# moldyn/Clustering

Measured on AMD Instinct MI355X. Metric: frame-pairs/s (density pop+nn), higher is better.
Workload: dtype f32 (Gram form on two fp16 pieces per coordinate on the f16 MFMA pipe, f32 accumulate, as a classifier with a guard band; undecided pairs re-checked in canonical f32)

## Files before the change

clustering_amd/csrc/dc_mfma.hip:

```cpp
#include "dc_mfma_kernels.hpp"
#include "dc_against.hpp"
#include "dc_against_nn.hpp"

#include <algorithm>
#include <cstring>
#include <atomic>
#include <mutex>

#ifndef DC_STEP_MASK
#define DC_STEP_MASK 0xFFFFu
#endif

namespace dc {

namespace {

#include "dc_mfma32.hpp"

__global__ void colsum_kernel(const float* __restrict__ coords, uint32_t n_rows, uint32_t D,
                              double* __restrict__ sums) {
  __shared__ double part[kMaxCols];
  if (threadIdx.x < (uint32_t)kMaxCols) part[threadIdx.x] = 0.0;
  __syncthreads();
  const uint32_t nthreads = gridDim.x * blockDim.x;
// ... 880 lines not shown
    const char* v;
    if ((v = env("DC_POP_SYM"))) w.pop_sym = v[0] != '0';
    if ((v = env("DC_POP_SHARED"))) w.pop_shared = atoi(v);
    if ((v = env("DC_NN_SHARED"))) w.nn_shared = atoi(v);
    w.waves_per_group = one_of_124(env("DC_WAVES_PER_GROUP"), 0);
    if ((v = env("DC_NN_COOP"))) w.nn_coop = atoi(v);
    if ((v = env("DC_NN_RHO"))) w.nn_rho = v[0] != '0';
    if ((v = env("DC_WAVE_TARGET"))) w.wave_target = (uint32_t)atoi(v);
    if ((v = env("DC_SHARE_FLOOR"))) w.share_floor = (uint32_t)atoi(v);
    if ((v = env("DC_POP_COMPONENTS"))) w.components = v[0] != '0';
    w.pop_cell_frames = (v = env("DC_POP_CELL_FRAMES")) ? (float)atof(v) : kPopCellFrames;
    w.nn_cell_frames = (v = env("DC_NN_CELL_FRAMES")) ? (float)atof(v) : kNnCellFrames;
    if ((v = env("DC_NN_FE_BITS"))) w.nn_fe_bits = atoi(v);
    w.mfma32_wpb = (uint32_t)one_of_124(env("DC_MFMA32_WPB"), 1);
    if ((v = env("DC_MFMA32_CHUNKS"))) w.mfma32_chunks = (uint32_t)atoi(v);
    return w;
  }();
  return sw;
}

static float cell_frames(bool nn) { return nn ? sweep_switches().nn_cell_frames : sweep_switches().pop_cell_frames; }
static float nn_cell_frames() { return cell_frames(true); }

int mfma_prepare(const float* d_coords, uint32_t n_rows, uint32_t n_cols, void* d_ws, hipStream_t stream,
                 bool stats_valid, bool pruned, const float* d_fe) {
  char* p = (char*)d_ws;
  const uint32_t cookie = data_cookie(d_coords, n_rows, n_cols);
  if (stats_valid) {
    const Layout L = make_layout(n_rows, n_cols);
    const size_t total = (size_t)n_rows * n_cols;
    const uint32_t B = (uint32_t)std::max<size_t>(1, std::min<size_t>(kClaimBlocks, (total + 1023) / 1024));
    unsigned long long* tab = (unsigned long long*)(p + L.fixed_end);
    const bool nn_reuse = pruned && d_fe != nullptr;
// ... 1163 lines not shown
```

clustering_amd/csrc/dc_mfma.hpp:

```cpp
#pragma once
#include "dc_common.hpp"

namespace dc {

struct EdgeSink {
  uint2* edges;
  unsigned long long* count;
  unsigned long long capacity;
  const uint32_t* comp;
  const uint32_t* rank;
  unsigned long long* best;
};
enum SinkMode { kSinkNone = 0, kSinkPairs = 1, kSinkMinEdge = 2 };

struct SweepSwitches {
  bool pop_sym = true;
  int pop_shared = -1;
  int nn_shared = -1;
  int waves_per_group = 0;
  int nn_coop = -1;
  bool nn_rho = true;
  uint32_t wave_target = 0;
  uint32_t share_floor = 0;
  bool components = true;
  float pop_cell_frames = 0.0f;
  float nn_cell_frames = 0.0f;
  int nn_fe_bits = -1;
  uint32_t mfma32_wpb = 1;
  uint32_t mfma32_chunks = 0;
};
const SweepSwitches& sweep_switches();

enum PopForm {
  kPopWave,
  kPopWaveSym,
  kPopPairs,
  kPopMinEdge,
  kPopShared,
  kPopSharedSym,
  kPopMsym,
  kPopMulti,
};
enum NnForm {
  kNnWave,
  kNnShared,
};
// ... 131 lines not shown
```

clustering_amd/csrc/dc_mfma_kernels.hpp:

```cpp
#pragma once
#include "dc_mfma.hpp"
#include "dc_credit.hpp"
#include "dc_rho_gap.hpp"
#include "dc_wide_prune.hpp"

#include <assert.h>
#include <float.h>
#include <math.h>
#include <stdlib.h>

#include <type_traits>

namespace dc {

namespace {

typedef float f32x16 __attribute__((ext_vector_type(16)));
typedef short s16x8 __attribute__((ext_vector_type(8)));

constexpr int kMaxCols = 64;
constexpr int kConstSlots = 2;
constexpr int kPieceGroups = 3;
constexpr int nm_for(int n_cols) { return (kPieceGroups * n_cols + kConstSlots + 15) / 16; }
constexpr int kMaxMfma = nm_for(kMaxCols);
// ... 175 lines not shown
  float cinv;
  int g, a, rounded;
};
constexpr uint32_t kHdrScale = 20;
constexpr uint32_t kHdrFp = 14;
constexpr uint32_t kHdrCookie = 28;
constexpr uint32_t kHdrMused = 31;
constexpr uint32_t kHdrOpen = 30;
constexpr uint32_t kHdrMfmaPop = 6, kHdrMfmaNn = 26;
constexpr uint32_t kHdrLayoutBad = 18;
constexpr uint32_t kHdrShares = 19;
constexpr uint32_t kHdrStatsBlocks = 25;
constexpr int kMfmaCtrPop = (kHdrMfmaPop - 2) / 2, kMfmaCtrNn = (kHdrMfmaNn - 4) / 2;
constexpr uint32_t kHdrShift = 32;
constexpr uint32_t kHdrMloc = 29;
constexpr int kMidShiftPop = 6, kConstShiftPop = 6, kConstShiftNn = 15;
constexpr float kThrCapPop = 1048576.0f;

__host__ __device__ inline Scale make_scale(const ScaleExp& e) {
  Scale s;
  s.sa = e.c;
  s.sb = e.c;
  s.s2 = e.s2;
  s.up = ldexpf(1.0f, e.g);
  s.dn = ldexpf(1.0f, -e.g);
  s.cinv = ldexpf(1.0f, -e.a);
  s.g = e.g;
  s.a = e.a;
  s.rounded = e.rounded;
  return s;
// ... 501 lines not shown
#pragma unroll
    for (int rr = 0; rr < NR; ++rr) {
      const uint32_t total = q[qt].cnt[rr] + (uint32_t)__shfl_xor((int)q[qt].cnt[rr], 32, 64);
      if (h == 0 && live && rr < n_rad) {
        if constexpr (M == kSelf) {
          const float dself = exact_d2(X.qcoords, n_cols, jq[qt], jq[qt]);
          pops[(size_t)rr * X.n_q + jq[qt]] = total + 1u - ((dself < rad2.v[rr]) ? 1u : 0u);
        } else {
          pops[(size_t)rr * X.n_q + jq[qt]] = total;
        }
      }
    }
  }
}

__device__ __forceinline__ uint32_t xcd_block(uint32_t n_blocks) {
  const uint32_t b = blockIdx.x, phys = b & 7u, idx = b >> 3;
  const uint32_t eighth = (phys + blockIdx.y) & 7u;
  const uint32_t n_full = n_blocks >> 3, rem = n_blocks & 7u;
  if (idx >= n_full + (eighth < rem ? 1u : 0u)) return 0xFFFFFFFFu;
  return eighth * n_full + min(eighth, rem) + idx;
}
inline uint32_t grid_x8(uint32_t n_blocks) { return (n_blocks + 7u) & ~7u; }

enum QueryMode { kQueryOwnOrder = 0, kQueryAll = 1 };

constexpr int kListCap = 512;
constexpr int kQueueCap = 4;
constexpr int kWaveQueue = 128;
constexpr int kSeedNeighbours = 4;

constexpr uint32_t kPopQueuePosBits = 24;
constexpr uint32_t kPopQueueMaxRows = 1u << kPopQueuePosBits;
static_assert(kMinEdgeMaxRows + kOrderPadRows == kPopQueueMaxRows, "min-edge sweeps take the queue path only");
static_assert(kOrderPadRows == (size_t)32 * kPadTiles, "pad positions of the orders");

__device__ __forceinline__ void emit_edge(const EdgeSink& sink, bool have, uint32_t pos_q, uint32_t pos_r) {
  const uint64_t m = __builtin_amdgcn_ballot_w64(have);
// ... 144 lines not shown
        if (e0 + 64u * j < total) dst[e0 + 64u * j] = v[j];
    }
  } else if (lane < 32) {
    const float* x = coords + (size_t)frame * n_cols;
    for (uint32_t k0 = 0; k0 < n_cols; k0 += 4) {
      float v[4];
#pragma unroll
      for (uint32_t j = 0; j < 4; ++j) v[j] = (live && k0 + j < n_cols) ? x[k0 + j] : 0.0f;
#pragma unroll
      for (uint32_t j = 0; j < 4; ++j)
        if (k0 + j < n_cols) dst[(uint32_t)lane * n_cols + k0 + j] = v[j];
    }
  }
}

template <int NM, int NR, int TQ, int MODE = kSinkNone, bool SYM = false>
__global__ __launch_bounds__(256, 2) void pop_pruned_kernel(
    const float* __restrict__ coords, uint32_t n_rows, uint32_t n_cols,
    const uint4* __restrict__ img_r, const float* __restrict__ norms_r,
    const uint32_t* __restrict__ perm_r, const float4* __restrict__ box_r,
    const float* __restrict__ coords_r, uint32_t T,
    const uint4* __restrict__ img_q, const float* __restrict__ norms_q,
    const uint32_t* __restrict__ perm_q, const float4* __restrict__ box_q, uint32_t n_q, QSeg q_seg,
    const uint32_t* __restrict__ hdr, unsigned long long* __restrict__ chain_counter, Rad2 rad2,
    int n_rad, uint32_t* __restrict__ pops, EdgeSink sink, CompView CV, uint32_t* __restrict__ pops_pos = nullptr) {
  static_assert(!SYM || (MODE == kSinkNone && NR == 1), "the symmetric sweep is the plain one-radius sweep");
  extern __shared__ __attribute__((aligned(16))) float pop_dyn_lds[];
  if (hdr[1] != 0) return;
  const int lane = threadIdx.x & 63, h = lane >> 5, c = lane & 31;
  const int wib = threadIdx.x >> 6;
  const uint32_t wpb = blockDim.x >> 6;
  uint32_t* lists_all = reinterpret_cast<uint32_t*>(pop_dyn_lds);
  float* pop_qrows_all = pop_dyn_lds + (size_t)wpb * kListCap;
  const uint32_t TQT = (n_q + 31) / 32;
  const uint32_t blk_unit = xcd_block((seg_groups((TQT + TQ - 1) / TQ, q_seg) + wpb - 1) / wpb);
  if (blk_unit == 0xFFFFFFFFu) return;
  const uint32_t wave = seg_group(blk_unit * wpb + wib, q_seg);
  const uint32_t chunk = blockIdx.y, n_chunks = gridDim.y;
  const uint32_t qt0 = wave * TQ;
  if (qt0 >= TQT) return;
  const uint32_t my_comp = CV.tile_comp_q[qt0];
  const uint32_t comp_lo = CV.range_r[2 * my_comp], comp_hi = CV.range_r[2 * my_comp + 1];
  uint32_t* list = lists_all + (size_t)wib * kListCap;
  float* qrows = pop_qrows_all + (size_t)wib * (TQ * 32) * n_cols;
  uint32_t* queues = reinterpret_cast<uint32_t*>(pop_qrows_all + (size_t)wpb * (TQ * 32) * n_cols) +
                     (size_t)wib * TQ * kQueueCap * 64;
  const bool use_queue = CV.n_pos <= kPopQueueMaxRows;
  constexpr bool kWaveWide = (MODE == kSinkNone) && (NR == 1) && (TQ * 32 <= 256) && (TQ * kQueueCap * 64 >= kWaveQueue + TQ * 32);
  uint32_t* fix_tab = queues + kWaveQueue;
  uint32_t qn = 0;
  uint32_t qcount[TQ];
  uint32_t comp_q[TQ], rank_q[TQ];
  unsigned long long edge_key[TQ];
// ... 339 lines not shown
        if (chunk == 0) {
          const float dself = exact_d2(coords, n_cols, jq[qt], jq[qt]);
          v += 1u - ((dself < rad2.v[rr]) ? 1u : 0u);
        }
        if constexpr (SYM)
          atomicAdd(&pops_pos[(qt0 + (uint32_t)qt) * 32u + (uint32_t)c], v);
        else if (n_chunks == 1)
          pops[(size_t)rr * n_rows + jq[qt]] = v;
        else
          atomicAdd(&pops[(size_t)rr * n_rows + jq[qt]], v);
      }
    }
  }
}


#include "dc_mfma_shared.hpp"
#include "dc_mfma_msym.hpp"

__device__ __forceinline__ void lexi_update(bool cond, float& bd, uint32_t& bj, float d,
                                            uint32_t j, uint32_t n_rows) {
  const bool take = cond & ((d < bd) | ((d == bd) & (j < bj) & (bj <= n_rows)));
  bd = take ? d : bd;
  bj = take ? j : bj;
}

struct NnQ {
  float m_nn, m_hd;
  float bd_nn, bd_hd;
  uint32_t bj_nn, bj_hd;
// ... 341 lines not shown
    const short one = live ? (short)const_a_bits(sc.a) : (short)0;
    b[0][0] = one;
    b[0][1] = one;
  }
}
template <int NM>
__device__ __forceinline__ void load_tile_folded(const uint4* __restrict__ img, uint32_t t, int lane, s16x8 (&a)[NM]) {
  const uint4* ip = img + (size_t)t * (NM * 64) + lane;
#pragma unroll
  for (int m = 0; m < NM; ++m) {
    const uint4 v = ip[m * 64];
    a[m] = __builtin_bit_cast(s16x8, v);
  }
}

template <int NM, int TQ, bool COOP = false>
__global__ __launch_bounds__(COOP ? 512 : 256, COOP ? 1 : 2) void nn_pruned_kernel(
    const float* __restrict__ coords, uint32_t n_rows, uint32_t n_cols,
    const float* __restrict__ fe, const uint4* __restrict__ img_r,
    const float* __restrict__ norms_r, const uint32_t* __restrict__ perm_r,
    const float4* __restrict__ box_r, const float4* __restrict__ box_t,
    const float2* __restrict__ rho_r, const float2* __restrict__ rho_t,
    const float2* __restrict__ ferange_r,
    const float* __restrict__ fe_c, const float* __restrict__ coords_c,
    const uint32_t* __restrict__ invpos_r, uint32_t T,
    const uint4* __restrict__ img_q, const float* __restrict__ norms_q,
    const uint32_t* __restrict__ perm_q, const float4* __restrict__ box_q, uint32_t n_q, QSeg q_seg,
    int full_range, float cell2,
    const uint32_t* __restrict__ hdr, unsigned long long* __restrict__ chain_counter,
    unsigned long long* __restrict__ merge64, uint32_t* __restrict__ nn_idx,
    float* __restrict__ nn_d2, uint32_t* __restrict__ hd_idx, float* __restrict__ hd_d2, CompView CV) {
  extern __shared__ __attribute__((aligned(16))) float nn_dyn_lds[];
  if (hdr[1] != 0) return;
  const int lane = threadIdx.x & 63, h = lane >> 5, c = lane & 31;
  const int wib = threadIdx.x >> 6;
  const uint32_t wpb = blockDim.x >> 6;
  uint32_t* lists_all = reinterpret_cast<uint32_t*>(nn_dyn_lds);
  float* qrows_all = nn_dyn_lds + (size_t)wpb * kListCap;
  const uint32_t TQT = (n_q + 31) / 32;
  const uint32_t blk_unit = xcd_block(COOP ? seg_groups((TQT + TQ - 1) / TQ, q_seg) : (seg_groups((TQT + TQ - 1) / TQ, q_seg) + wpb - 1) / wpb);
  if (blk_unit == 0xFFFFFFFFu) return;
  const uint32_t wave = seg_group(COOP ? blk_unit : blk_unit * wpb + wib, q_seg);
  const uint32_t chunk = COOP ? blockIdx.y * wpb + (uint32_t)wib : blockIdx.y, n_chunks = COOP ? gridDim.y * wpb : gridDim.y;
  const uint32_t qt0 = wave * TQ;
  if (qt0 >= TQT) return;
  const uint32_t my_comp = CV.tile_comp_q[qt0];
  const uint32_t comp_lo = CV.range_r[2 * my_comp], comp_hi = CV.range_r[2 * my_comp + 1];
  const float comp_cell = __uint_as_float(CV.comp[kCompFine + 4 * min(my_comp, (uint32_t)kMaxComp - 1u) + 2]);
  uint32_t* list = lists_all + (size_t)wib * kListCap;
  uint32_t* coop_base = lists_all + (size_t)wpb * kListCap;
  float* qrows = COOP ? reinterpret_cast<float*>(coop_base + (size_t)wpb * 2 * kWaveQueue + 8 * TQ * 32)
                      : qrows_all + (size_t)wib * (TQ * 32) * n_cols;
  uint32_t* queues = COOP ? coop_base + (size_t)wib * 2 * kWaveQueue
                          : reinterpret_cast<uint32_t*>(qrows_all + (size_t)wpb * (TQ * 32) * n_cols) +
                                (size_t)wib * (TQ * kQueueCap * 64 + 2 * TQ * 32);
  static_assert(TQ * kQueueCap * 64 >= 2 * kWaveQueue + 4 * TQ * 32, "candidate list + incumbents fit the queue region");
  uint2* cand = reinterpret_cast<uint2*>(queues);
  unsigned long long* best64 = reinterpret_cast<unsigned long long*>(COOP ? coop_base + (size_t)wpb * 2 * kWaveQueue : queues + 2 * kWaveQueue);
// ... 70 lines not shown
        for (uint32_t j = 0; j < 8; ++j) v[j] = (e0 + nthr * j < total) ? src[e0 + nthr * j] : 0.0f;
#pragma unroll
        for (uint32_t j = 0; j < 8; ++j)
          if (e0 + nthr * j < total) qrows[e0 + nthr * j] = v[j];
      }
    } else {
#pragma unroll
      for (int qt = 0; qt < TQ; ++qt) {
        if (((uint32_t)qt % wpb) != (uint32_t)wib) continue;
        const uint32_t tile = qt0 + qt, tl = tile < TQT ? tile : TQT - 1;
        stage_query_rows(qrows + (size_t)qt * 32 * n_cols, full_range ? coords_c + (size_t)tl * 32 * n_cols : nullptr, coords,
                         jq[qt], (livemask[qt] >> lane) & 1, n_cols, lane);
      }
    }
    __syncthreads();
    if (blockIdx.y == 0) {
#pragma unroll
      for (int qt = 0; qt < TQ; ++qt) {
        const bool live = (livemask[qt] >> lane) & 1;
        float bd_nn = FLT_MAX, bd_hd = FLT_MAX;
        uint32_t bj_nn = n_rows + 1, bj_hd = n_rows + 1;
        if (live) {
          const float* qrow = qrows + (qt * 32 + c) * n_cols;
          for (int k = 1 + wib; k <= kSeedNeighbours; k += (int)wpb) {
            const long long p2 = (long long)q[qt].spos + (h ? -k : k);
            if (p2 >= 0 && p2 < (long long)CV.n_pos && perm_r[p2] != kInvalidFrame) {
              const float d2c = dist2_canon_rt(qrow, 1, coords_c + (size_t)p2 * n_cols, 1, (int)n_cols);
              const uint32_t j = perm_r[p2];
              lexi_update(true, bd_nn, bj_nn, d2c, j, n_rows);
              lexi_update(fe_c[p2] < q[qt].feq, bd_hd, bj_hd, d2c, j, n_rows);
            }
// ... 488 lines not shown
      jq[qt] = perm_q[(qt0 + qt) * 32 + c];
      const unsigned long long w_nn = best64[qt * 32 + c], w_hd = best64[TQ * 32 + qt * 32 + c];
      if (n_chunks == 1) {
        nn_idx[jq[qt]] = (uint32_t)w_nn;
        nn_d2[jq[qt]] = __uint_as_float((uint32_t)(w_nn >> 32));
        hd_idx[jq[qt]] = (uint32_t)w_hd;
        hd_d2[jq[qt]] = __uint_as_float((uint32_t)(w_hd >> 32));
      } else {
        atomicMin(&merge64[jq[qt]], w_nn);
        atomicMin(&merge64[(size_t)n_rows + jq[qt]], w_hd);
      }
    }
  }
}

#include "dc_mfma_nn_shared.hpp"

__global__ void nn_merge_fill_kernel(unsigned long long* __restrict__ merge64, uint32_t n_rows) {
  const uint32_t i = blockIdx.x * blockDim.x + threadIdx.x;
  if (i < 2 * n_rows) merge64[i] = ((unsigned long long)__float_as_uint(FLT_MAX) << 32) | (n_rows + 1);
}

__global__ void nn_merge_unpack_kernel(const unsigned long long* __restrict__ merge64,
                                       const uint32_t* __restrict__ perm_q, uint32_t n_q,
                                       uint32_t n_rows, uint32_t tq, QSeg q_seg,
                                       uint32_t* __restrict__ nn_idx, float* __restrict__ nn_d2,
                                       uint32_t* __restrict__ hd_idx, float* __restrict__ hd_d2) {
  const uint32_t p = blockIdx.x * blockDim.x + threadIdx.x;
  if (p >= n_q) return;
  if (!seg_owns(p / (32u * tq), q_seg)) return;
// ... 34 lines not shown
  return (waves + 3) / 4;
}

template <int S, SweepMode M>
void pop_dispatch(const SweepArgs& X, uint32_t n_cols, uint32_t i_from, uint32_t i_to, const Rad2& rad2, uint32_t* pops,
                  hipStream_t s) {
  constexpr int kTQ = tq_full_for<S>;
  const dim3 grid(grid_for(i_from, i_to, kTQ)), block(256);
  sweep_timer_mark(0, true, s);
  hipLaunchKernelGGL((pop_mfma_kernel<S, 1, kTQ, M>), grid, block, 0, s, X, n_cols, i_from, i_to, rad2, 1, pops);
  sweep_timer_mark(0, false, s);
}

__global__ void box_by_share_kernel(const float4* __restrict__ box_r, uint32_t T, uint32_t n_chunks,
                                    float4* __restrict__ box_t, const float2* __restrict__ rho_r,
                                    float2* __restrict__ rho_t) {
  const uint32_t t = blockIdx.x * blockDim.x + threadIdx.x;
  if (t >= T) return;
  const uint32_t stride = (T + n_chunks - 1) / n_chunks;
  box_t[(size_t)(t % n_chunks) * stride + t / n_chunks] = box_r[t];
  if (rho_r) rho_t[(size_t)(t % n_chunks) * stride + t / n_chunks] = rho_r[t];
}

struct NnPrunedArgs {
  const uint4* img_r;
  const float* norms_r;
  const uint32_t* perm_r;
  const float4* box_r;
  float4* box_t;
  const float2* rho_r;
  float2* rho_t;
  const float2* ferange_r;
// ... 97 lines not shown
  if (sw.share_floor) share_floor = sw.share_floor;
  const uint32_t waves = (tiles + tq - 1) / tq;
  uint32_t r = waves >= target ? 1u : (target + waves - 1) / waves;
  const uint32_t by_share = ref_tiles / share_floor;
  const uint32_t cap = by_share < 64u ? by_share : 64u;
  r = r > cap ? cap : r;
  return r < 1u ? 1u : r;
}

template <class F>
void timed_launch(int kind, hipStream_t s, F&& launch) {
  sweep_timer_mark(kind, true, s);
  launch();
  sweep_timer_mark(kind, false, s);
}
inline void nn_shares_begin(const NnPrunedArgs& A, uint32_t n_rows, uint32_t T, uint32_t n_chunks, bool with_rho, hipStream_t s) {
  if (n_chunks > 1)
    hipLaunchKernelGGL(nn_merge_fill_kernel, dim3((2 * n_rows + 255) / 256), dim3(256), 0, s, A.merge64, n_rows);
  hipLaunchKernelGGL(box_by_share_kernel, dim3((T + 255) / 256), dim3(256), 0, s, A.box_r, T, n_chunks, A.box_t,
                     with_rho ? A.rho_r : (const float2*)nullptr, A.rho_t);
}
inline void nn_shares_end(const NnPrunedArgs& A, uint32_t n_rows, uint32_t n_chunks, uint32_t group_tiles,
                          uint32_t* nn_idx, float* nn_d2, uint32_t* hd_idx, float* hd_d2, hipStream_t s) {
  if (n_chunks <= 1) return;
  if (A.full_range)
    hipLaunchKernelGGL(nn_merge_unpack_rows_kernel, dim3((n_rows + 255) / 256), dim3(256), 0, s,
                       (const unsigned long long*)A.merge64, A.invpos_r, n_rows, group_tiles, A.q_seg, nn_idx, nn_d2,
                       hd_idx, hd_d2);
  else
    hipLaunchKernelGGL(nn_merge_unpack_kernel, dim3((A.n_q + 255) / 256), dim3(256), 0, s,
                       (const unsigned long long*)A.merge64, A.perm_q, A.n_q, n_rows, group_tiles, A.q_seg, nn_idx,
                       nn_d2, hd_idx, hd_d2);
}

template <int S>
// ... 28 lines not shown
          launch(std::integral_constant<int, kNbMin>{});
        else
          launch(std::integral_constant<int, kNbMax>{});
      } else {
        launch(std::integral_constant<int, kNbMax>{});
      }
      nn_shares_end(A, n_rows, n_chunks, 4u * TQV, nn_idx, nn_d2, hd_idx, hd_d2, s);
    }
    return;
  }
  constexpr int TQV = tq_nn(S);
  assert(pl.tq == (uint32_t)TQV);
  const uint32_t waves = seg_groups(((A.n_q + 31) / 32 + TQV - 1) / TQV, A.q_seg), tiles = waves * TQV;
  if (waves == 0) return;
  uint32_t n_chunks = pick_chunks(tiles, TQV, kNnWaveTargetPerWave, T, kNnShareFloor, (size_t)S * 1024 + 128);
  if (n_chunks >= pl.coop_shares) {
    n_chunks = (n_chunks + kNnCoopWaves - 1) / kNnCoopWaves * kNnCoopWaves;
    const size_t smem_c = sizeof(uint32_t) * (kNnCoopWaves * (kListCap + 2 * kWaveQueue) + 8 * TQV * 32) +
                          sizeof(float) * TQV * 32 * (size_t)n_cols;
    nn_shares_begin(A, n_rows, T, n_chunks, true, s);
    timed_launch(1, s, [&] {
      hipLaunchKernelGGL((nn_pruned_kernel<S, TQV, true>), dim3(grid_x8(waves), n_chunks / kNnCoopWaves), dim3(64 * kNnCoopWaves), smem_c, s,
                         coords, n_rows, n_cols, fe, A.img_r, A.norms_r, A.perm_r, A.box_r, (const float4*)A.box_t, A.rho_r,
                         (const float2*)(A.rho_r ? A.rho_t : nullptr), A.ferange_r, A.fe_c, A.coords_c, A.invpos_r, T, A.img_q, A.norms_q, A.perm_q, A.box_q, A.n_q, A.q_seg,
                         A.full_range, A.cell2, hdr, chain_counter, A.merge64, nn_idx, nn_d2, hd_idx, hd_d2, CV);
    });
  } else {
    const uint32_t wpb = pl.waves;
    const size_t smem = wpb * (sizeof(uint32_t) * kListCap + sizeof(float) * TQV * 32 * (size_t)n_cols +
                               sizeof(uint32_t) * (TQV * kQueueCap * 64 + 2 * TQV * 32));
    nn_shares_begin(A, n_rows, T, n_chunks, true, s);
    timed_launch(1, s, [&] {
      hipLaunchKernelGGL((nn_pruned_kernel<S, TQV>), dim3(grid_x8((waves + wpb - 1) / wpb), n_chunks), dim3(64 * wpb), smem, s,
                         coords, n_rows, n_cols, fe, A.img_r, A.norms_r, A.perm_r, A.box_r, (const float4*)A.box_t, A.rho_r,
                         (const float2*)(A.rho_r ? A.rho_t : nullptr), A.ferange_r, A.fe_c, A.coords_c, A.invpos_r, T, A.img_q, A.norms_q, A.perm_q, A.box_q, A.n_q, A.q_seg,
                         A.full_range, A.cell2, hdr, chain_counter, A.merge64, nn_idx, nn_d2, hd_idx, hd_d2, CV);
    });
  }
  nn_shares_end(A, n_rows, n_chunks, (uint32_t)TQV, nn_idx, nn_d2, hd_idx, hd_d2, s);
}

__global__ void pops_by_frame_kernel(const uint32_t* __restrict__ pops_pos, const uint32_t* __restrict__ perm,
                                     uint32_t n_rows, const uint32_t* __restrict__ hdr, uint32_t* __restrict__ pops) {
  if (hdr[1] != 0) return;
  const uint32_t pos = blockIdx.x * blockDim.x + threadIdx.x;
  if (pos < n_rows && perm[pos] != kInvalidFrame) pops[perm[pos]] = pops_pos[pos];
}

template <int S>
void pop_pruned_dispatch(const PopPlan& pl, const float* coords, uint32_t n_rows, uint32_t n_cols, const Ptrs& P,
                         uint32_t T, uint32_t n_q, int q_mode, QSeg q_seg, const Rad2& rad2,
// ... 68 lines not shown
        else
          shared(std::integral_constant<int, 8>{});
      }
      return;
    case kPopShared:
    case kPopSharedSym:
      if constexpr (pop_form_built(kPopShared, S)) shared(std::integral_constant<int, 1>{});
      return;
    default:
      break;
  }
  constexpr int TQ = tq_pop(S);
  assert(pl.tq == (uint32_t)TQ);
  const uint32_t waves = seg_groups(((n_q + 31) / 32 + TQ - 1) / TQ, q_seg), tiles = waves * TQ;
  if (waves == 0) return;
  const uint32_t wpb = pl.waves;
  const dim3 grid(grid_x8((waves + wpb - 1) / wpb), pick_chunks(tiles, TQ, kPopWaveTarget, T, pop_share_floor(T), (size_t)S * 1024 + 128)),
      block(64 * wpb);
  const size_t smem = wpb * (sizeof(uint32_t) * kListCap + sizeof(float) * TQ * 32 * (size_t)n_cols +
                             sizeof(uint32_t) * TQ * kQueueCap * 64);
  const EdgeSink no_sink{nullptr, nullptr, 0, nullptr, nullptr, nullptr};
  auto launch = [&](auto mode_c, auto sym_c, uint32_t* pops_pos) {
    timed_launch(0, s, [&] {
      hipLaunchKernelGGL((pop_pruned_kernel<S, 1, TQ, decltype(mode_c)::value, decltype(sym_c)::value>), grid, block, smem, s,
                         coords, n_rows, n_cols, P.img_p, P.norms_p, P.perm_p, P.box_p, P.coords_p, T, img_q, norms_q,
                         perm_q, box_q, n_q, q_seg, P.hdr, chain_counter, rad2, n_rad, pops, sink ? *sink : no_sink, CV,
                         pops_pos);
    });
  };
  switch (pl.form) {
    case kPopWaveSym: {
      uint32_t* pops_pos = const_cast<uint32_t*>(P.pq);
      if (!pos_clean) (void)hipMemsetAsync(pops_pos, 0, sizeof(uint32_t) * 32 * (size_t)T, s);
      launch(std::integral_constant<int, kSinkNone>{}, std::true_type{}, pops_pos);
      cross((uint32_t)TQ, pops_pos, (size_t)32 * T, 1);
      hipLaunchKernelGGL(pops_by_frame_kernel, dim3((32 * T + 255) / 256), dim3(256), 0, s, (const uint32_t*)pops_pos,
                         P.perm_p, 32u * T, P.hdr, pops);
      return;
    }
    case kPopMinEdge: launch(std::integral_constant<int, kSinkMinEdge>{}, std::false_type{}, nullptr); break;
    case kPopPairs: launch(std::integral_constant<int, kSinkPairs>{}, std::false_type{}, nullptr); break;
    default: launch(std::integral_constant<int, kSinkNone>{}, std::false_type{}, nullptr); break;
  }
// ... 32 lines not shown
```

clustering_amd/csrc/dc_prep.hpp:

```cpp
#pragma once

constexpr float kStatsLimit = 5.0e16f;

constexpr uint32_t kStatsRow = kMaxCols + 3;
constexpr uint32_t kStatsMaxBlocks = 2048;
__global__ __launch_bounds__(256) void stats_kernel(const float* __restrict__ coords, uint32_t n_rows, uint32_t D,
                                                    uint32_t* __restrict__ hdr, uint32_t cookie, double* __restrict__ table) {
  __shared__ double part[kMaxCols];
  __shared__ uint32_t wave_max[4];
  __shared__ unsigned long long fp_part[4];
  if (threadIdx.x < (uint32_t)kMaxCols) part[threadIdx.x] = 0.0;
  __syncthreads();
  const uint32_t nthreads = gridDim.x * blockDim.x;
  const uint32_t used = (nthreads / D) * D;
  const uint32_t id = blockIdx.x * blockDim.x + threadIdx.x;
  const size_t total = (size_t)n_rows * D;
  const uint32_t* w = reinterpret_cast<const uint32_t*>(coords);
  const uint32_t col = id % D;
  double s0 = 0.0, s1 = 0.0, s2 = 0.0, s3 = 0.0;
  uint32_t m_lo = 0, m_hi = 0;
  unsigned long long fp = 0;
  bool bad = false;
  auto take = [&](uint32_t bits, size_t e, double& s) {
    const float v = __uint_as_float(bits);
// ... 499 lines not shown
    float* __restrict__ coords_o, float4* __restrict__ boxes, const float* __restrict__ fe, float* __restrict__ fe_s,
    uint32_t* __restrict__ invpos, float2* __restrict__ ferange, float2* __restrict__ rhorange,
    const uint32_t* __restrict__ tile_comp,
    const float* __restrict__ origins, uint32_t* __restrict__ hdr, uint4* __restrict__ img_a, int a_form,
    float* __restrict__ norms_a, uint4* __restrict__ img_b, float* __restrict__ norms_b, uint32_t grp_tq, QSeg grp,
    unsigned long long* __restrict__ hash_slots, uint32_t* __restrict__ zero_pos, uint32_t zero_planes) {
  extern __shared__ float or_tile[];
  __shared__ uint32_t s_frame[256];
  __shared__ unsigned long long fp_part[4];
  const uint32_t Dp = D | 1u;
  const uint32_t pos0 = blockIdx.x * 256u, pos = pos0 + threadIdx.x, n_pos = 32u * T;
  const uint32_t frame = (pos < n_pos) ? perm[pos] : kInvalidFrame;
  s_frame[threadIdx.x] = frame;
  if (zero_pos && pos < n_pos)
    for (uint32_t z = 0; z < zero_planes; ++z) zero_pos[(size_t)z * n_pos + pos] = 0u;
  __syncthreads();
  const size_t base = (size_t)pos0 * D, total = (size_t)n_pos * D;
  for (uint32_t e0 = threadIdx.x; e0 < 256u * D; e0 += 1024u) {
    float v[4];
    uint32_t off[4];
#pragma unroll
    for (uint32_t j = 0; j < 4; ++j) {
      const uint32_t e = e0 + 256u * j;
      const uint32_t r = min(e / D, 255u), k = e - (e / D) * D;
      const uint32_t i = s_frame[r];
      off[j] = r * Dp + k;
      v[j] = (e < 256u * D && i != kInvalidFrame) ? coords[(size_t)i * D + k] : 0.0f;
    }
#pragma unroll
    for (uint32_t j = 0; j < 4; ++j) {
// ... 213 lines not shown
```

Baseline: 93140 billion.

## Replace static sweep grid with persistent blocks drawing work tickets per XCD queue

The pop and nn pruned sweep kernels now run as persistent blocks sized to resident occupancy. Each block pulls (block, share) work units from eight atomic ticket counters, one per XCD-aligned queue, and steals from the other queues once its own runs dry. The aim is to fix load imbalance across uneven pruned work and to cut the cost of launching many short-lived blocks. In exchange the kernels gain atomics, extra barriers and ticket-reset steps, and correctness depends on the counters being zeroed before every launch.

```diff
diff --git a/clustering_amd/csrc/dc_mfma.hip b/clustering_amd/csrc/dc_mfma.hip
--- a/clustering_amd/csrc/dc_mfma.hip
+++ b/clustering_amd/csrc/dc_mfma.hip
@@ -6,6 +6,7 @@
 #include <cstring>
 #include <atomic>
 #include <mutex>
+#include <vector>
 
 #ifndef DC_STEP_MASK
 #define DC_STEP_MASK 0xFFFFu
@@ -918,9 +919,37 @@
     if ((v = env("DC_NN_FE_BITS"))) w.nn_fe_bits = atoi(v);
     w.mfma32_wpb = (uint32_t)one_of_124(env("DC_MFMA32_WPB"), 1);
     if ((v = env("DC_MFMA32_CHUNKS"))) w.mfma32_chunks = (uint32_t)atoi(v);
+    if ((v = env("DC_SWEEP_DISPATCH"))) w.tickets = strcmp(v, "static") != 0;
+    if ((v = env("DC_SWEEP_SLOTS"))) w.sweep_slots = (uint32_t)std::max(atoi(v), 0);
     return w;
   }();
   return sw;
+}
+
+uint32_t sweep_resident_slots(const void* kernel, uint32_t block_threads, size_t dyn_lds) {
+  struct Entry {
+    int dev;
+    const void* kernel;
+    uint32_t block;
+    size_t lds;
+    uint32_t slots;
+  };
+  static std::mutex mu;
+  static std::vector<Entry> known;
+  int dev = 0;
+  (void)hipGetDevice(&dev);
+  std::lock_guard<std::mutex> lock(mu);
+  for (const Entry& e : known)
+    if (e.dev == dev && e.kernel == kernel && e.block == block_threads && e.lds == dyn_lds) return e.slots;
+  int per_cu = 0, cus = 0;
+  if (hipOccupancyMaxActiveBlocksPerMultiprocessor(&per_cu, kernel, (int)block_threads, dyn_lds) != hipSuccess || per_cu < 1 ||
+      hipDeviceGetAttribute(&cus, hipDeviceAttributeMultiprocessorCount, dev) != hipSuccess || cus < 1) {
+    (void)hipGetLastError();
+    per_cu = 1;
+    cus = 8;
+  }
+  known.push_back(Entry{dev, kernel, block_threads, dyn_lds, (uint32_t)per_cu * (uint32_t)cus});
+  return known.back().slots;
 }
 
 static float cell_frames(bool nn) { return nn ? sweep_switches().nn_cell_frames : sweep_switches().pop_cell_frames; }
diff --git a/clustering_amd/csrc/dc_mfma.hpp b/clustering_amd/csrc/dc_mfma.hpp
--- a/clustering_amd/csrc/dc_mfma.hpp
+++ b/clustering_amd/csrc/dc_mfma.hpp
@@ -28,8 +28,11 @@
   int nn_fe_bits = -1;
   uint32_t mfma32_wpb = 1;
   uint32_t mfma32_chunks = 0;
+  bool tickets = true;
+  uint32_t sweep_slots = 0;
 };
 const SweepSwitches& sweep_switches();
+uint32_t sweep_resident_slots(const void* kernel, uint32_t block_threads, size_t dyn_lds);
 
 enum PopForm {
   kPopWave,
diff --git a/clustering_amd/csrc/dc_mfma_kernels.hpp b/clustering_amd/csrc/dc_mfma_kernels.hpp
--- a/clustering_amd/csrc/dc_mfma_kernels.hpp
+++ b/clustering_amd/csrc/dc_mfma_kernels.hpp
@@ -3,6 +3,7 @@
 #include "dc_credit.hpp"
 #include "dc_rho_gap.hpp"
 #include "dc_wide_prune.hpp"
+#include "dc_sweep_units.hpp"
 
 #include <assert.h>
 #include <float.h>
@@ -213,6 +214,8 @@
 constexpr int kMfmaCtrPop = (kHdrMfmaPop - 2) / 2, kMfmaCtrNn = (kHdrMfmaNn - 4) / 2;
 constexpr uint32_t kHdrShift = 32;
 constexpr uint32_t kHdrMloc = 29;
+constexpr uint32_t kHdrTicketsPop = 40, kHdrTicketsNn = 48;
+static_assert(4 * (kHdrTicketsNn + 8) <= kHdrSums && kHdrTicketsPop > kHdrShift, "ticket counters in the free header words");
 constexpr int kMidShiftPop = 6, kConstShiftPop = 6, kConstShiftNn = 15;
 constexpr float kThrCapPop = 1048576.0f;
 
@@ -744,14 +747,75 @@
   }
 }
 
-__device__ __forceinline__ uint32_t xcd_block(uint32_t n_blocks) {
-  const uint32_t b = blockIdx.x, phys = b & 7u, idx = b >> 3;
-  const uint32_t eighth = (phys + blockIdx.y) & 7u;
-  const uint32_t n_full = n_blocks >> 3, rem = n_blocks & 7u;
-  if (idx >= n_full + (eighth < rem ? 1u : 0u)) return 0xFFFFFFFFu;
-  return eighth * n_full + min(eighth, rem) + idx;
-}
+__device__ __forceinline__ uint32_t xcd_block(uint32_t n_blocks) { return xcd_unit(n_blocks, blockIdx.x, blockIdx.y); }
 inline uint32_t grid_x8(uint32_t n_blocks) { return (n_blocks + 7u) & ~7u; }
+
+struct SweepTickets {
+  uint32_t* ctr;
+  uint32_t n_chunks;
+};
+__device__ __forceinline__ SweepUnit draw_unit(uint32_t* __restrict__ ctr, uint32_t n_blocks, uint32_t n_chunks, uint32_t& k,
+                                               bool first_lane) {
+  while (k < kSweepQueues) {
+    const uint32_t qq = (blockIdx.x + k) & 7u;
+    uint32_t t = 0;
+    if (first_lane) t = atomicAdd(&ctr[qq], 1u);
+    const SweepUnit u = sweep_unit(n_blocks, n_chunks, qq, (uint32_t)__builtin_amdgcn_readfirstlane((int)t));
+    if (u.blk != kNoUnit) return u;
+    ++k;
+  }
+  return SweepUnit{kNoUnit, 0u};
+}
+template <class A>
+__device__ __forceinline__ const A* kernargs_again() {
+  auto* p = (const __attribute__((address_space(4))) A*)__builtin_amdgcn_kernarg_segment_ptr();
+  asm volatile("" : "+s"(p));
+  return (const A*)p;
+}
+__device__ __forceinline__ uint32_t thread_again() {
+  uint32_t t = threadIdx.x;
+  asm volatile("" : "+v"(t));
+  return t;
+}
+template <class A, class NBlocks, class Body>
+__device__ __forceinline__ void for_each_unit(uint32_t* slot, NBlocks&& n_blocks_of, Body&& body) {
+  for (uint32_t k = 0;;) {
+    const A& a = *kernargs_again<A>();
+    const uint32_t n_blocks = n_blocks_of(a);
+    uint32_t blk, share, shares;
+    if (a.tk.ctr == nullptr) {
+      if (k != 0) return;
+      k = kSweepQueues;
+      blk = xcd_block(n_blocks);
+      share = blockIdx.y;
+      shares = gridDim.y;
+    } else {
+      shares = a.tk.n_chunks;
+      const uint32_t tid = thread_again();
+      const bool first_lane = (tid & 63u) == 0;
+      if (blockDim.x == 64u) {
+        const SweepUnit u = draw_unit(a.tk.ctr, n_blocks, shares, k, first_lane);
+        blk = u.blk;
+        share = u.share;
+      } else {
+        __syncthreads();
+        if (__builtin_amdgcn_readfirstlane((int)(tid >> 6)) == 0) {
+          const SweepUnit u = draw_unit(a.tk.ctr, n_blocks, shares, k, first_lane);
+          if (first_lane) {
+            slot[0] = u.blk;
+            slot[1] = u.share;
+          }
+        }
+        __syncthreads();
+        blk = (uint32_t)__builtin_amdgcn_readfirstlane((int)slot[0]);
+        share = (uint32_t)__builtin_amdgcn_readfirstlane((int)slot[1]);
+        __syncthreads();
+      }
+    }
+    if (blk == kNoUnit) return;
+    body(a, blk, share, shares);
+  }
+}
 
 enum QueryMode { kQueryOwnOrder = 0, kQueryAll = 1 };
 
@@ -926,8 +990,9 @@
   }
 }
 
-template <int NM, int NR, int TQ, int MODE = kSinkNone, bool SYM = false>
-__global__ __launch_bounds__(256, 2) void pop_pruned_kernel(
+template <int NM, int NR, int TQ, int MODE, bool SYM>
+__device__ __forceinline__ void pop_pruned_unit(
+    uint32_t blk_unit, uint32_t chunk, uint32_t n_chunks, float* __restrict__ pop_dyn_lds,
     const float* __restrict__ coords, uint32_t n_rows, uint32_t n_cols,
     const uint4* __restrict__ img_r, const float* __restrict__ norms_r,
     const uint32_t* __restrict__ perm_r, const float4* __restrict__ box_r,
@@ -935,20 +1000,16 @@
     const uint4* __restrict__ img_q, const float* __restrict__ norms_q,
     const uint32_t* __restrict__ perm_q, const float4* __restrict__ box_q, uint32_t n_q, QSeg q_seg,
     const uint32_t* __restrict__ hdr, unsigned long long* __restrict__ chain_counter, Rad2 rad2,
-    int n_rad, uint32_t* __restrict__ pops, EdgeSink sink, CompView CV, uint32_t* __restrict__ pops_pos = nullptr) {
+    int n_rad, uint32_t* __restrict__ pops, EdgeSink sink, CompView CV, uint32_t* __restrict__ pops_pos) {
   static_assert(!SYM || (MODE == kSinkNone && NR == 1), "the symmetric sweep is the plain one-radius sweep");
-  extern __shared__ __attribute__((aligned(16))) float pop_dyn_lds[];
-  if (hdr[1] != 0) return;
-  const int lane = threadIdx.x & 63, h = lane >> 5, c = lane & 31;
-  const int wib = threadIdx.x >> 6;
+  const uint32_t tid = thread_again();
+  const int lane = tid & 63, h = lane >> 5, c = lane & 31;
+  const int wib = __builtin_amdgcn_readfirstlane((int)(tid >> 6));
   const uint32_t wpb = blockDim.x >> 6;
   uint32_t* lists_all = reinterpret_cast<uint32_t*>(pop_dyn_lds);
   float* pop_qrows_all = pop_dyn_lds + (size_t)wpb * kListCap;
   const uint32_t TQT = (n_q + 31) / 32;
-  const uint32_t blk_unit = xcd_block((seg_groups((TQT + TQ - 1) / TQ, q_seg) + wpb - 1) / wpb);
-  if (blk_unit == 0xFFFFFFFFu) return;
   const uint32_t wave = seg_group(blk_unit * wpb + wib, q_seg);
-  const uint32_t chunk = blockIdx.y, n_chunks = gridDim.y;
   const uint32_t qt0 = wave * TQ;
   if (qt0 >= TQT) return;
   const uint32_t my_comp = CV.tile_comp_q[qt0];
@@ -1318,6 +1379,48 @@
   }
 }
 
+struct PopKernArgs {
+  const float* coords;
+  uint32_t n_rows, n_cols;
+  const uint4* img_r;
+  const float* norms_r;
+  const uint32_t* perm_r;
+  const float4* box_r;
+  const float* coords_r;
+  uint32_t T;
+  const uint4* img_q;
+  const float* norms_q;
+  const uint32_t* perm_q;
+  const float4* box_q;
+  uint32_t n_q;
+  QSeg q_seg;
+  const uint32_t* hdr;
+  unsigned long long* chain_counter;
+  Rad2 rad2;
+  int n_rad;
+  uint32_t* pops;
+  EdgeSink sink;
+  CompView CV;
+  uint32_t* pops_pos;
+  SweepTickets tk;
+};
+template <int NM, int NR, int TQ, int MODE = kSinkNone, bool SYM = false>
+__global__ __launch_bounds__(256, 2) void pop_pruned_kernel(PopKernArgs A0) {
+  extern __shared__ __attribute__((aligned(16))) float pop_dyn_lds[];
+  if (A0.hdr[1] != 0) return;
+  for_each_unit<PopKernArgs>(
+      reinterpret_cast<uint32_t*>(pop_dyn_lds),
+      [](const PopKernArgs& A) {
+        const uint32_t wpb = blockDim.x >> 6;
+        return (seg_groups(((A.n_q + 31) / 32 + TQ - 1) / TQ, A.q_seg) + wpb - 1) / wpb;
+      },
+      [&](const PopKernArgs& A, uint32_t blk_unit, uint32_t chunk, uint32_t n_chunks) {
+        pop_pruned_unit<NM, NR, TQ, MODE, SYM>(blk_unit, chunk, n_chunks, pop_dyn_lds, A.coords, A.n_rows, A.n_cols, A.img_r, A.norms_r,
+                                               A.perm_r, A.box_r, A.coords_r, A.T, A.img_q, A.norms_q, A.perm_q, A.box_q, A.n_q,
+                                               A.q_seg, A.hdr, A.chain_counter, A.rad2, A.n_rad, A.pops, A.sink, A.CV, A.pops_pos);
+      });
+}
+
 
 #include "dc_mfma_shared.hpp"
 #include "dc_mfma_msym.hpp"
@@ -1689,8 +1792,9 @@
   }
 }
 
-template <int NM, int TQ, bool COOP = false>
-__global__ __launch_bounds__(COOP ? 512 : 256, COOP ? 1 : 2) void nn_pruned_kernel(
+template <int NM, int TQ, bool COOP>
+__device__ __forceinline__ void nn_pruned_unit(
+    uint32_t blk_unit, uint32_t share_y, uint32_t n_shares_y, float* __restrict__ nn_dyn_lds,
     const float* __restrict__ coords, uint32_t n_rows, uint32_t n_cols,
     const float* __restrict__ fe, const uint4* __restrict__ img_r,
     const float* __restrict__ norms_r, const uint32_t* __restrict__ perm_r,
@@ -1705,18 +1809,15 @@
     const uint32_t* __restrict__ hdr, unsigned long long* __restrict__ chain_counter,
     unsigned long long* __restrict__ merge64, uint32_t* __restrict__ nn_idx,
     float* __restrict__ nn_d2, uint32_t* __restrict__ hd_idx, float* __restrict__ hd_d2, CompView CV) {
-  extern __shared__ __attribute__((aligned(16))) float nn_dyn_lds[];
-  if (hdr[1] != 0) return;
-  const int lane = threadIdx.x & 63, h = lane >> 5, c = lane & 31;
-  const int wib = threadIdx.x >> 6;
+  const uint32_t tid = thread_again();
+  const int lane = tid & 63, h = lane >> 5, c = lane & 31;
+  const int wib = __builtin_amdgcn_readfirstlane((int)(tid >> 6));
   const uint32_t wpb = blockDim.x >> 6;
   uint32_t* lists_all = reinterpret_cast<uint32_t*>(nn_dyn_lds);
   float* qrows_all = nn_dyn_lds + (size_t)wpb * kListCap;
   const uint32_t TQT = (n_q + 31) / 32;
-  const uint32_t blk_unit = xcd_block(COOP ? seg_groups((TQT + TQ - 1) / TQ, q_seg) : (seg_groups((TQT + TQ - 1) / TQ, q_seg) + wpb - 1) / wpb);
-  if (blk_unit == 0xFFFFFFFFu) return;
   const uint32_t wave = seg_group(COOP ? blk_unit : blk_unit * wpb + wib, q_seg);
-  const uint32_t chunk = COOP ? blockIdx.y * wpb + (uint32_t)wib : blockIdx.y, n_chunks = COOP ? gridDim.y * wpb : gridDim.y;
+  const uint32_t chunk = COOP ? share_y * wpb + (uint32_t)wib : share_y, n_chunks = COOP ? n_shares_y * wpb : n_shares_y;
   const uint32_t qt0 = wave * TQ;
   if (qt0 >= TQT) return;
   const uint32_t my_comp = CV.tile_comp_q[qt0];
@@ -1817,7 +1918,7 @@
       }
     }
     __syncthreads();
-    if (blockIdx.y == 0) {
+    if (share_y == 0) {
 #pragma unroll
       for (int qt = 0; qt < TQ; ++qt) {
         const bool live = (livemask[qt] >> lane) & 1;
@@ -2336,6 +2437,61 @@
   }
 }
 
+struct NnKernArgs {
+  const float* coords;
+  uint32_t n_rows, n_cols;
+  const float* fe;
+  const uint4* img_r;
+  const float* norms_r;
+  const uint32_t* perm_r;
+  const float4 *box_r, *box_t;
+  const float2 *rho_r, *rho_t, *ferange_r;
+  const float *fe_c, *coords_c;
+  const uint32_t* invpos_r;
+  uint32_t T;
+  const uint4* img_q;
+  const float* norms_q;
+  const uint32_t* perm_q;
+  const float4* box_q;
+  uint32_t n_q;
+  QSeg q_seg;
+  int full_range;
+  float cell2;
+  const uint32_t* hdr;
+  unsigned long long* chain_counter;
+  unsigned long long* merge64;
+  uint32_t* nn_idx;
+  float* nn_d2;
+  uint32_t* hd_idx;
+  float* hd_d2;
+  CompView CV;
+  SweepTickets tk;
+};
+template <int NM, int TQ, bool COOP = false>
+__global__ __launch_bounds__(COOP ? 512 : 256, COOP ? 1 : 2) void nn_pruned_kernel(NnKernArgs A0) {
+  extern __shared__ __attribute__((aligned(16))) float nn_dyn_lds[];
+  if (A0.hdr[1] != 0) return;
+  auto groups_of = [](const NnKernArgs& A) { return seg_groups(((A.n_q + 31) / 32 + TQ - 1) / TQ, A.q_seg); };
+  auto unit = [&](const NnKernArgs& A, uint32_t blk_unit, uint32_t share_y, uint32_t n_shares_y) {
+    nn_pruned_unit<NM, TQ, COOP>(blk_unit, share_y, n_shares_y, nn_dyn_lds, A.coords, A.n_rows, A.n_cols, A.fe, A.img_r, A.norms_r,
+                                 A.perm_r, A.box_r, A.box_t, A.rho_r, A.rho_t, A.ferange_r, A.fe_c, A.coords_c, A.invpos_r, A.T, A.img_q,
+                                 A.norms_q, A.perm_q, A.box_q, A.n_q, A.q_seg, A.full_range, A.cell2, A.hdr, A.chain_counter, A.merge64,
+                                 A.nn_idx, A.nn_d2, A.hd_idx, A.hd_d2, A.CV);
+  };
+  if constexpr (COOP) {
+    const uint32_t blk_unit = xcd_block(groups_of(A0));
+    if (blk_unit != kNoUnit) unit(A0, blk_unit, blockIdx.y, gridDim.y);
+  } else {
+    for_each_unit<NnKernArgs>(
+        reinterpret_cast<uint32_t*>(nn_dyn_lds),
+        [&](const NnKernArgs& A) {
+          const uint32_t wpb = blockDim.x >> 6;
+          return (groups_of(A) + wpb - 1) / wpb;
+        },
+        unit);
+  }
+}
+
 #include "dc_mfma_nn_shared.hpp"
 
 __global__ void nn_merge_fill_kernel(unsigned long long* __restrict__ merge64, uint32_t n_rows) {
@@ -2400,8 +2556,9 @@
 
 __global__ void box_by_share_kernel(const float4* __restrict__ box_r, uint32_t T, uint32_t n_chunks,
                                     float4* __restrict__ box_t, const float2* __restrict__ rho_r,
-                                    float2* __restrict__ rho_t) {
+                                    float2* __restrict__ rho_t, uint32_t* __restrict__ tickets) {
   const uint32_t t = blockIdx.x * blockDim.x + threadIdx.x;
+  if (tickets && t < kSweepQueues) tickets[t] = 0u;
   if (t >= T) return;
   const uint32_t stride = (T + n_chunks - 1) / n_chunks;
   box_t[(size_t)(t % n_chunks) * stride + t / n_chunks] = box_r[t];
@@ -2529,11 +2686,21 @@
   launch();
   sweep_timer_mark(kind, false, s);
 }
-inline void nn_shares_begin(const NnPrunedArgs& A, uint32_t n_rows, uint32_t T, uint32_t n_chunks, bool with_rho, hipStream_t s) {
+inline void nn_shares_begin(const NnPrunedArgs& A, uint32_t n_rows, uint32_t T, uint32_t n_chunks, bool with_rho, hipStream_t s,
+                            uint32_t* tickets = nullptr) {
   if (n_chunks > 1)
     hipLaunchKernelGGL(nn_merge_fill_kernel, dim3((2 * n_rows + 255) / 256), dim3(256), 0, s, A.merge64, n_rows);
   hipLaunchKernelGGL(box_by_share_kernel, dim3((T + 255) / 256), dim3(256), 0, s, A.box_r, T, n_chunks, A.box_t,
-                     with_rho ? A.rho_r : (const float2*)nullptr, A.rho_t);
+                     with_rho ? A.rho_r : (const float2*)nullptr, A.rho_t, tickets);
+}
+inline dim3 ticket_grid(const void* kernel, uint32_t block_threads, size_t dyn_lds, uint32_t n_blocks, uint32_t n_chunks,
+                        const SweepSwitches& sw) {
+  uint32_t g = sweep_resident_slots(kernel, block_threads, dyn_lds);
+  if (sw.sweep_slots != 0 && sw.sweep_slots < g) g = sw.sweep_slots;
+  const unsigned long long units = (unsigned long long)n_blocks * n_chunks;
+  if (units < g) g = (uint32_t)units;
+  if (g >= kSweepQueues) g &= ~(kSweepQueues - 1u);
+  return dim3(g < 1u ? 1u : g);
 }
 inline void nn_shares_end(const NnPrunedArgs& A, uint32_t n_rows, uint32_t n_chunks, uint32_t group_tiles,
                           uint32_t* nn_idx, float* nn_d2, uint32_t* hd_idx, float* hd_d2, hipStream_t s) {
@@ -2592,6 +2759,12 @@
   const uint32_t waves = seg_groups(((A.n_q + 31) / 32 + TQV - 1) / TQV, A.q_seg), tiles = waves * TQV;
   if (waves == 0) return;
   uint32_t n_chunks = pick_chunks(tiles, TQV, kNnWaveTargetPerWave, T, kNnShareFloor, (size_t)S * 1024 + 128);
+  auto kern_args = [&](const SweepTickets& tk) {
+    return NnKernArgs{coords, n_rows, n_cols, fe, A.img_r, A.norms_r, A.perm_r, A.box_r, (const float4*)A.box_t, A.rho_r,
+                      (const float2*)(A.rho_r ? A.rho_t : nullptr), A.ferange_r, A.fe_c, A.coords_c, A.invpos_r, T, A.img_q,
+                      A.norms_q, A.perm_q, A.box_q, A.n_q, A.q_seg, A.full_range, A.cell2, hdr, chain_counter, A.merge64,
+                      nn_idx, nn_d2, hd_idx, hd_d2, CV, tk};
+  };
   if (n_chunks >= pl.coop_shares) {
     n_chunks = (n_chunks + kNnCoopWaves - 1) / kNnCoopWaves * kNnCoopWaves;
     const size_t smem_c = sizeof(uint32_t) * (kNnCoopWaves * (kListCap + 2 * kWaveQueue) + 8 * TQV * 32) +
@@ -2599,20 +2772,19 @@
     nn_shares_begin(A, n_rows, T, n_chunks, true, s);
     timed_launch(1, s, [&] {
       hipLaunchKernelGGL((nn_pruned_kernel<S, TQV, true>), dim3(grid_x8(waves), n_chunks / kNnCoopWaves), dim3(64 * kNnCoopWaves), smem_c, s,
-                         coords, n_rows, n_cols, fe, A.img_r, A.norms_r, A.perm_r, A.box_r, (const float4*)A.box_t, A.rho_r,
-                         (const float2*)(A.rho_r ? A.rho_t : nullptr), A.ferange_r, A.fe_c, A.coords_c, A.invpos_r, T, A.img_q, A.norms_q, A.perm_q, A.box_q, A.n_q, A.q_seg,
-                         A.full_range, A.cell2, hdr, chain_counter, A.merge64, nn_idx, nn_d2, hd_idx, hd_d2, CV);
+                         kern_args(SweepTickets{nullptr, 0u}));
     });
   } else {
-    const uint32_t wpb = pl.waves;
+    const uint32_t wpb = pl.waves, n_blocks = (waves + wpb - 1) / wpb;
     const size_t smem = wpb * (sizeof(uint32_t) * kListCap + sizeof(float) * TQV * 32 * (size_t)n_cols +
                                sizeof(uint32_t) * (TQV * kQueueCap * 64 + 2 * TQV * 32));
-    nn_shares_begin(A, n_rows, T, n_chunks, true, s);
+    const SweepSwitches& sw = sweep_switches();
+    const SweepTickets tk{sw.tickets ? const_cast<uint32_t*>(hdr) + kHdrTicketsNn : nullptr, n_chunks};
+    const dim3 grid = tk.ctr ? ticket_grid((const void*)&nn_pruned_kernel<S, TQV>, 64 * wpb, smem, n_blocks, n_chunks, sw)
+                             : dim3(grid_x8(n_blocks), n_chunks);
+    nn_shares_begin(A, n_rows, T, n_chunks, true, s, tk.ctr);
     timed_launch(1, s, [&] {
-      hipLaunchKernelGGL((nn_pruned_kernel<S, TQV>), dim3(grid_x8((waves + wpb - 1) / wpb), n_chunks), dim3(64 * wpb), smem, s,
-                         coords, n_rows, n_cols, fe, A.img_r, A.norms_r, A.perm_r, A.box_r, (const float4*)A.box_t, A.rho_r,
-                         (const float2*)(A.rho_r ? A.rho_t : nullptr), A.ferange_r, A.fe_c, A.coords_c, A.invpos_r, T, A.img_q, A.norms_q, A.perm_q, A.box_q, A.n_q, A.q_seg,
-                         A.full_range, A.cell2, hdr, chain_counter, A.merge64, nn_idx, nn_d2, hd_idx, hd_d2, CV);
+      hipLaunchKernelGGL((nn_pruned_kernel<S, TQV>), grid, dim3(64 * wpb), smem, s, kern_args(tk));
     });
   }
   nn_shares_end(A, n_rows, n_chunks, (uint32_t)TQV, nn_idx, nn_d2, hd_idx, hd_d2, s);
@@ -2711,19 +2883,22 @@
   assert(pl.tq == (uint32_t)TQ);
   const uint32_t waves = seg_groups(((n_q + 31) / 32 + TQ - 1) / TQ, q_seg), tiles = waves * TQ;
   if (waves == 0) return;
-  const uint32_t wpb = pl.waves;
-  const dim3 grid(grid_x8((waves + wpb - 1) / wpb), pick_chunks(tiles, TQ, kPopWaveTarget, T, pop_share_floor(T), (size_t)S * 1024 + 128)),
-      block(64 * wpb);
+  const uint32_t wpb = pl.waves, n_blocks = (waves + wpb - 1) / wpb;
+  const uint32_t n_chunks = pick_chunks(tiles, TQ, kPopWaveTarget, T, pop_share_floor(T), (size_t)S * 1024 + 128);
+  const dim3 block(64 * wpb);
   const size_t smem = wpb * (sizeof(uint32_t) * kListCap + sizeof(float) * TQ * 32 * (size_t)n_cols +
                              sizeof(uint32_t) * TQ * kQueueCap * 64);
   const EdgeSink no_sink{nullptr, nullptr, 0, nullptr, nullptr, nullptr};
+  const SweepSwitches& sw = sweep_switches();
+  const SweepTickets tk{sw.tickets ? const_cast<uint32_t*>(P.hdr) + kHdrTicketsPop : nullptr, n_chunks};
   auto launch = [&](auto mode_c, auto sym_c, uint32_t* pops_pos) {
-    timed_launch(0, s, [&] {
-      hipLaunchKernelGGL((pop_pruned_kernel<S, 1, TQ, decltype(mode_c)::value, decltype(sym_c)::value>), grid, block, smem, s,
-                         coords, n_rows, n_cols, P.img_p, P.norms_p, P.perm_p, P.box_p, P.coords_p, T, img_q, norms_q,
-                         perm_q, box_q, n_q, q_seg, P.hdr, chain_counter, rad2, n_rad, pops, sink ? *sink : no_sink, CV,
-                         pops_pos);
-    });
+    auto kernel = &pop_pruned_kernel<S, 1, TQ, decltype(mode_c)::value, decltype(sym_c)::value>;
+    const dim3 grid = tk.ctr ? ticket_grid((const void*)kernel, block.x, smem, n_blocks, n_chunks, sw) : dim3(grid_x8(n_blocks), n_chunks);
+    if (tk.ctr && !pos_clean) (void)hipMemsetAsync(tk.ctr, 0, sizeof(uint32_t) * kSweepQueues, s);
+    const PopKernArgs args{coords, n_rows, n_cols, P.img_p, P.norms_p, P.perm_p, P.box_p, P.coords_p, T, img_q, norms_q,
+                           perm_q, box_q, n_q, q_seg, P.hdr, chain_counter, rad2, n_rad, pops, sink ? *sink : no_sink, CV,
+                           pops_pos, tk};
+    timed_launch(0, s, [&] { hipLaunchKernelGGL(kernel, grid, block, smem, s, args); });
   };
   switch (pl.form) {
     case kPopWaveSym: {
diff --git a/clustering_amd/csrc/dc_prep.hpp b/clustering_amd/csrc/dc_prep.hpp
--- a/clustering_amd/csrc/dc_prep.hpp
+++ b/clustering_amd/csrc/dc_prep.hpp
@@ -537,6 +537,7 @@
   s_frame[threadIdx.x] = frame;
   if (zero_pos && pos < n_pos)
     for (uint32_t z = 0; z < zero_planes; ++z) zero_pos[(size_t)z * n_pos + pos] = 0u;
+  if (zero_pos && pos < kSweepQueues) hdr[kHdrTicketsPop + pos] = 0u;
   __syncthreads();
   const size_t base = (size_t)pos0 * D, total = (size_t)n_pos * D;
   for (uint32_t e0 = threadIdx.x; e0 < 256u * D; e0 += 1024u) {
diff --git a/clustering_amd/csrc/dc_sweep_units.hpp b/clustering_amd/csrc/dc_sweep_units.hpp
--- /dev/null
+++ b/clustering_amd/csrc/dc_sweep_units.hpp
@@ -0,0 +1,50 @@
+#pragma once
+#include <stdint.h>
+
+#if defined(__HIPCC__) || defined(__CUDACC__)
+#define DC_UNITS_FN __host__ __device__ __forceinline__
+#else
+#define DC_UNITS_FN inline
+#endif
+
+constexpr uint32_t kNoUnit = 0xFFFFFFFFu;
+constexpr uint32_t kSweepQueues = 8;
+
+DC_UNITS_FN uint32_t eighth_len(uint32_t n_blocks, uint32_t e) { return (n_blocks >> 3) + (e < (n_blocks & 7u) ? 1u : 0u); }
+DC_UNITS_FN uint32_t eighth_first(uint32_t n_blocks, uint32_t e) {
+  const uint32_t rem = n_blocks & 7u;
+  return e * (n_blocks >> 3) + (e < rem ? e : rem);
+}
+
+DC_UNITS_FN uint32_t xcd_unit(uint32_t n_blocks, uint32_t bx, uint32_t by) {
+  const uint32_t phys = bx & 7u, idx = bx >> 3;
+  const uint32_t eighth = (phys + by) & 7u;
+  if (idx >= eighth_len(n_blocks, eighth)) return kNoUnit;
+  return eighth_first(n_blocks, eighth) + idx;
+}
+
+struct SweepUnit {
+  uint32_t blk, share;
+};
+DC_UNITS_FN uint32_t sweep_queue_len(uint32_t n_blocks, uint32_t n_chunks, uint32_t q) {
+  uint32_t len = (n_chunks >> 3) * n_blocks;
+  for (uint32_t y = n_chunks & ~7u; y < n_chunks; ++y) len += eighth_len(n_blocks, (q + y) & 7u);
+  return len;
+}
+DC_UNITS_FN SweepUnit sweep_unit(uint32_t n_blocks, uint32_t n_chunks, uint32_t q, uint32_t ticket) {
+  SweepUnit u{kNoUnit, 0u};
+  if (n_blocks == 0) return u;
+  const uint32_t cyc = ticket / n_blocks;
+  uint32_t r = ticket - cyc * n_blocks;
+  if (cyc >= (n_chunks + 7u) >> 3) return u;
+  for (uint32_t y = 8u * cyc; y < n_chunks; ++y) {
+    const uint32_t e = (q + y) & 7u, len = eighth_len(n_blocks, e);
+    if (r < len) {
+      u.blk = eighth_first(n_blocks, e) + r;
+      u.share = y;
+      return u;
+    }
+    r -= len;
+  }
+  return u;
+}
```

New measurement: 100100 billion (median of 6 runs). +7.5%, better.
